# ConsenSys/gnark-crypto

Hardware: AMD Instinct MI355X
Metric: G1 MSM/sec (BN254) (higher is better)
Workload: dtype u32; 1 GPU; BN254 G1 MultiExp 2^20 points, bases+scalars resident in HBM; points=1048576, window_bits=16, windows=8, glv_half_scalars=True, resident_bases=False, parallelism=single GPU

## Files before the change

gnark-crypto_amd/csrc/gmsm_context.h:

```cpp
#pragma once
#include <hip/hip_runtime.h>
#include <atomic>

#include <algorithm>
#include <cstdio>
#include <cstdlib>
#include <chrono>
#include <condition_variable>
#include <memory>
#include <mutex>
#include <string>
#include <thread>
#include <vector>

#include "../../include/gmsm.h"

namespace gmsm {

int fail(int code, const std::string &msg);
void clear_last_error();

#define HIP_TRY(expr)                                                                                        \
    do {                                                                                                     \
        hipError_t e_ = (expr);                                                                              \
// ... 96 lines not shown
        for (auto *b : bufs) any = any || b->ptr;
        if (!any) return;
        int prev = 0;
        (void)hipGetDevice(&prev);
        if (device >= 0) (void)hipSetDevice(device);
        (void)hipDeviceSynchronize();
        for (auto *b : bufs)
            if (b->ptr) (void)hipFree(b->ptr);
        (void)hipSetDevice(prev);
    }
};

struct Workspace {
    hipStream_t stream = nullptr;
    DeviceBuffer upoints, skip;
    DeviceBuffer seg_lvl;
    DeviceBuffer seg_partials, seg_flags, seg_bucket;
    DeviceBuffer parted;
    DeviceBuffer heavy;
    DeviceBuffer long_pieces;
    DeviceBuffer small_sums, small_done;
    DeviceBuffer digits, sorted, blockhist, counts, starts, buckets, partials, totals;
    DeviceBuffer red_pre;
    DeviceBuffer carry;
    hipStream_t mstream = nullptr;
    hipEvent_t ev_buckets = nullptr, ev_merged = nullptr;
    hipStream_t cstream = nullptr;
    hipEvent_t ev_fork = nullptr, ev_conv = nullptr;
    bool conv_pending = false;
    hipEvent_t events[12] = {nullptr};
    bool timed = false;
    int timed_level = 0;
    void *pinned = nullptr;
    size_t pinned_cap = 0;
    DeviceBuffer h2d_points, h2d_scalars;
    DeviceBuffer raw_bytes, flagword;
    DeviceBuffer poly;
    DeviceBuffer lagrange;
    bool busy = false;
    bool ticket = false;
    bool pending = false;
    int pending_group = -1;
    unsigned pending_c = 0;
    uint32_t pending_nw = 0;
    uint32_t pending_gen = 0;
    std::shared_ptr<ResidentBases> bases_ref;
    hipEvent_t dep = nullptr;
    bool uncollected = false;
    hipEvent_t last_use = nullptr;
    hipStream_t last_stream = nullptr;
    bool pending_timed = false;
    size_t trim(size_t keep) {
        DeviceBuffer *all[] = {&upoints, &skip, &seg_lvl, &seg_partials, &seg_flags, &seg_bucket, &parted, &heavy, &long_pieces, &small_sums, &small_done, &digits, &sorted,
                               &blockhist, &counts, &starts, &buckets, &partials, &totals, &red_pre, &carry, &h2d_points,
                               &h2d_scalars, &raw_bytes, &flagword, &poly, &lagrange};
        size_t freed = 0;
        for (DeviceBuffer *b : all)
            if (b->cap > keep) freed += b->release();
        if (pinned && pinned_cap > keep) {
            (void)hipHostFree(pinned);
            pinned = nullptr;
            pinned_cap = 0;
        }
        return freed;
    }
    void destroy() {
        (void)trim(0);
        hipEvent_t *evs[] = {&ev_buckets, &ev_merged, &dep, &last_use, &ev_fork, &ev_conv};
        for (hipEvent_t *e : evs) {
            if (*e) (void)hipEventDestroy(*e);
            *e = nullptr;
        }
        for (auto &e : events) {
            if (e) (void)hipEventDestroy(e);
            e = nullptr;
        }
        if (stream) (void)hipStreamDestroy(stream);
// ... 440 lines not shown
```

gnark-crypto_amd/csrc/gmsm_group.h:

```cpp
#pragma once
#include <algorithm>
#include <cstdlib>
#include <cstring>
#include <thread>
#include <type_traits>
#include <vector>

#include "gmsm_context.h"
#include "gmsm_group_host.h"
#include "gmsm_kernels.h"
#include "gmsm_fixup_q.h"
#include "gmsm_small.h"
#include "gmsm_fixedbase.h"
#include "gmsm_ingest.h"
#include "gmsm_decompress.h"
#include "gmsm_fft.h"
#include "gmsm_poly.h"
#include "gmsm_shplonk.h"
#include "gmsm_fflonk.h"
#include "gmsm_group_fft.h"
#include "gmsm_scale.h"
#include "gmsm_ratio.h"

namespace gmsm {
// ... 332 lines not shown
                                                    "2^(44-c) points for c > 17): use a smaller c or split by point range"
                                                  : "more than 2^27 points in one pipeline run: split the window sums by point range "
                                                    "and add the sets (gmsm_fold_window_sets); the MultiExp entries do this themselves");
        const size_t fine_cnt_bytes = (size_t)4 << fbits;
        const uint32_t stage_cap = fine_cnt_bytes >= 156 * 1024 ? 0u
                                   : (uint32_t)std::min<size_t>(GMSM_TUNE(STAGE_CAP, part_log2 >= 15 ? 39000 : 24576),
                                                              (156 * 1024 - fine_cnt_bytes) / 4);
        if (stage_cap > 40u * 1024u) return fail(GMSM_ERR_ARG, "window geometry: staging slots beyond the fine sort's registers");
        if (fine_cnt_bytes + (size_t)stage_cap * 4 > 160 * 1024)
            return fail(GMSM_ERR_ARG, "window geometry: fine-sort counters exceed the LDS");
        const bool d16 = max_digit_code(plan) < 65536;
        const size_t dsz = d16 ? 2 : 4;

        if ((rc = ws.digits.ensure((size_t)nw * n * dsz))) return rc;
        if ((rc = ws.sorted.ensure((size_t)nw * n * 4))) return rc;
        if ((rc = ws.parted.ensure((size_t)nw * n * 4))) return rc;
        if ((rc = ws.starts.ensure((size_t)nw * (NB + 1) * 4))) return rc;
        if ((rc = ws.buckets.ensure((size_t)nw * NB * REC))) return rc;
        if ((rc = ws.partials.ensure((tot_blk + (size_t)nw * q.nblocks2) * 2 * REC))) return rc;
        const uint32_t T = (uint32_t)(((size_t)NB + ((size_t)1 << q.log2L) - 1) >> q.log2L);
        if ((rc = ws.red_pre.ensure((size_t)nw * T * 2 * REC))) return rc;
        if ((rc = ws.totals.ensure((size_t)nwd * sizeof(Ext)))) return rc;
        if ((rc = ws.ensure_pinned((size_t)nwd * sizeof(Ext)))) return rc;
        if ((rc = ws.blockhist.ensure((size_t)nw * pchunks * nparts * 4))) return rc;
        if ((rc = ws.counts.ensure((size_t)nw * (2 * nparts + 1) * 4))) return rc;
        if ((rc = ws.seg_partials.ensure(tot_thr * 2 * REC))) return rc;
        if ((rc = ws.seg_flags.ensure(tot_thr * 4))) return rc;
        if ((rc = ws.seg_bucket.ensure(tot_thr * 4))) return rc;
        const size_t list_cap = 2 * (tot_thr / FIX_MAXWALK + tot_thr / LONG_PIECE + nw + 16);
        if ((rc = ws.seg_lvl.ensure((size_t)nw * 4 + 16 + list_cap * sizeof(LongChain)))) return rc;
        uint32_t *long_flag = (uint32_t *)ws.seg_lvl.ptr;
        LongChain *long_list = (LongChain *)((char *)ws.seg_lvl.ptr + (((size_t)nw * 4 + 15) / 16) * 16);
        const size_t piece_sums_off = ((list_cap * 4 + 15) / 16) * 16;
        if ((rc = ws.long_pieces.ensure(piece_sums_off + list_cap * REC))) return rc;
        uint32_t *piece_done = (uint32_t *)ws.long_pieces.ptr;
        void *piece_sums = (char *)ws.long_pieces.ptr + piece_sums_off;
        const uint32_t hcap = (uint32_t)std::min<size_t>(nparts, n / ((size_t)stage_cap + 1) + 1);
        const uint32_t scap = (uint32_t)(n / HEAVY_SUB) + hcap;
        const size_t hparts_bytes = (((size_t)nw * hcap * sizeof(HeavyPart) + 15) / 16) * 16, hcount_bytes = (((size_t)nw * 8 + 4 + 15) / 16) * 16;
        if ((rc = ws.heavy.ensure(hparts_bytes + hcount_bytes + ((size_t)nw * scap << fbits) * 4))) return rc;
        HeavyPart *hparts = (HeavyPart *)ws.heavy.ptr;
        uint32_t *hcount = (uint32_t *)((char *)ws.heavy.ptr + hparts_bytes);
        uint32_t *subhist = (uint32_t *)((char *)ws.heavy.ptr + hparts_bytes + hcount_bytes);
        if (nw > HEAVY_MAX_WINDOWS) return fail(GMSM_ERR_ARG, "more than 256 windows in one pipeline run");
        const uint32_t heavy_wg = (uint32_t)std::min<size_t>((size_t)2 * ctx.num_cus, std::max<size_t>((size_t)nw * scap, 1));
        uint32_t *bh = (uint32_t *)ws.blockhist.ptr, *part_base = (uint32_t *)ws.counts.ptr;
// ... 6 lines not shown
        if ((rc = ctx.allow_lds((const void *)k_part_scatter<uint16_t, PART_CHUNK_BIG>, 152 * 1024))) return rc;
        if ((rc = ctx.allow_lds((const void *)k_part_scatter<uint32_t, PART_CHUNK_BIG>, 152 * 1024))) return rc;
        if ((rc = ctx.allow_lds((const void *)k_fine_sort<24>, 160 * 1024))) return rc;
        if ((rc = ctx.allow_lds((const void *)k_fine_sort<40>, 160 * 1024))) return rc;
        if ((rc = ctx.allow_lds((const void *)k_heavy_hist, 128 * 1024))) return rc;
        if ((rc = ctx.allow_lds((const void *)k_heavy_scan, 128 * 1024))) return rc;
        if ((rc = ctx.allow_lds((const void *)k_heavy_place, 128 * 1024))) return rc;
        if ((rc = ctx.allow_lds((const void *)k_fixup_long<U>, (int)(128 * sizeof(QRec<U>))))) return rc;
        if constexpr (FIXUP_QUAD)
            if ((rc = ctx.allow_lds((const void *)k_fixup_seg_q<U>, (int)(128 * sizeof(QRec<U>))))) return rc;
        if ((rc = ctx.allow_lds((const void *)k_combine_q<U, true, COMBINE_N>, (int)((2 * COMBINE_N + 1) * sizeof(QRec<U>))))) return rc;
        if constexpr (COMBINE_WE)
            if ((rc = ctx.allow_lds((const void *)k_combine_we<U, true>, (int)((2 * COMBINE_N + 1) * sizeof(QRec<U>))))) return rc;
        if constexpr (SERIAL_QUAD)
            if ((rc = ctx.allow_lds((const void *)k_reduce_serial_q<U, SERIAL_Q_QUADS>, (int)(3 * SERIAL_Q_QUADS * sizeof(QRec<U>))))) return rc;
        if ((rc = ctx.allow_lds((const void *)k_reduce2_q<U, true>, (int)(2 * RED2_TPB * sizeof(QRec<U>))))) return rc;

        StageTimer timer(ws, !buckets_only || time_range);
        ws.timed = timer.on;
        timer.mark(T_DECOMPOSE, stream);
        const uint8_t *skip = nullptr;
        const void *upoints = nullptr;
        bool forked = false;
        if (resident) {
            upoints = (const char *)(shared ? resident->tables.ptr : resident->upoints.ptr) + resident_offset * AFF_BYTES;
            skip = (const uint8_t *)resident->skip.ptr + resident_offset;
        } else {
            if ((rc = ws.upoints.ensure((glv ? 2 : 1) * n_points * AFF_BYTES))) return rc;
            forked = n_points >= FORK_CONVERT_MIN;
            if (forked && (rc = ws.side_stream(ws.cstream))) return rc;
            hipStream_t cs = forked ? ws.cstream : stream;
            if (forked) {
                HIP_TRY(hipEventRecord(ws.ev_fork, stream));
                HIP_TRY(hipStreamWaitEvent(cs, ws.ev_fork, 0));
            }
            if (glv)
                hipLaunchKernelGGL((k_convert_points_glv<U, Consts>), dim3((unsigned)((n_points + 255) / 256)), dim3(256), 0,
                                   cs, d_points, n_points, ws.upoints.ptr);
            else
                hipLaunchKernelGGL((k_convert_points<U>), dim3((unsigned)((n_points + 255) / 256)), dim3(256), 0,
                                   cs, d_points, n_points, ws.upoints.ptr, (uint8_t *)nullptr);
            if (forked) {
                ws.conv_pending = true;
                HIP_TRY(hipEventRecord(ws.ev_conv, cs));
            }
            upoints = ws.upoints.ptr;
// ... 12 lines not shown
                               (const uint16_t *)digits, n, nparts, fbits, pchunk_len, bh);
        else
            hipLaunchKernelGGL(k_part_hist<uint32_t>, dim3(pchunks, nw), dim3(1024), (size_t)nparts * 4, stream,
                               (const uint32_t *)digits, n, nparts, fbits, pchunk_len, bh);
        timer.mark(T_SCAN, stream);
        if ((size_t)((nparts + 31) / 32) * nw < (size_t)ctx.num_cus && pchunks >= 256)
            hipLaunchKernelGGL(k_part_colscan<32>, dim3((nparts + 31) / 32, nw), dim3(1024), 0, stream, bh, pchunks, nparts, part_pop, hcount + 2 * nw);
        else
            hipLaunchKernelGGL(k_part_colscan<8>, dim3((nparts + 31) / 32, nw), dim3(256), 0, stream, bh, pchunks, nparts, part_pop, hcount + 2 * nw);
        hipLaunchKernelGGL(k_part_rowscan, dim3(nw), dim3(1024), 0, stream, part_pop, nparts, part_base, long_flag, stage_cap, hparts,
                           hcount, hcap);
        timer.mark(T_SCATTER, stream);
        {
            const dim3 grid(pchunks, nw), block(1024);
#define GMSM_SCATTER(D, CH)                                                                                              \
    hipLaunchKernelGGL((k_part_scatter<D, CH>), grid, block, scatter_lds, stream, (const D *)digits, n, nparts, fbits, lidx, \
                       pchunk_len, bh, part_base, parted)
            if (d16 && !big_chunk) GMSM_SCATTER(uint16_t, PART_CHUNK);
            else if (d16) GMSM_SCATTER(uint16_t, PART_CHUNK_BIG);
            else if (!big_chunk) GMSM_SCATTER(uint32_t, PART_CHUNK);
            else GMSM_SCATTER(uint32_t, PART_CHUNK_BIG);
#undef GMSM_SCATTER
        }
        if (stage_cap <= 24u * 1024u)
            hipLaunchKernelGGL(k_fine_sort<24>, dim3(nparts, nw), dim3(1024), ((size_t)4 << fbits) + (size_t)stage_cap * 4, stream,
                               parted, n, NB, fbits, lidx, part_base, sorted, starts, stage_cap);
        else
            hipLaunchKernelGGL(k_fine_sort<40>, dim3(nparts, nw), dim3(1024), ((size_t)4 << fbits) + (size_t)stage_cap * 4, stream,
                               parted, n, NB, fbits, lidx, part_base, sorted, starts, stage_cap);
        if (n > stage_cap) {
            hipLaunchKernelGGL(k_heavy_hist, dim3(heavy_wg), dim3(1024), (size_t)4 << fbits, stream, parted, n, nw, nparts, fbits, lidx,
                               part_base, (const HeavyPart *)hparts, (const uint32_t *)hcount, hcap, scap, subhist);
            hipLaunchKernelGGL(k_heavy_scan, dim3(std::min<uint32_t>(hcap, 64u), nw), dim3(1024), (size_t)4 << fbits, stream, nparts, NB, fbits,
                               part_base, (const HeavyPart *)hparts, (const uint32_t *)hcount, hcap, scap, subhist, starts);
            hipLaunchKernelGGL(k_heavy_place, dim3(heavy_wg), dim3(1024), (size_t)4 << fbits, stream, parted, n, nw, nparts, fbits, lidx,
                               part_base, (const HeavyPart *)hparts, (const uint32_t *)hcount, hcap, scap, (const uint32_t *)subhist, sorted);
        }
        if (forked) {
            HIP_TRY(hipStreamWaitEvent(stream, ws.ev_conv, 0));
            ws.conv_pending = false;
        }
        const auto accumulate = [&](uint32_t k0, uint32_t nk, hipStream_t st) {
            const uint32_t *st_g = starts + (size_t)k0 * (NB + 1);
            const uint32_t *sorted_g = sorted + (size_t)k0 * n;
            char *buckets_g = buckets + (size_t)k0 * NB * REC, *part_g = seg_partials + (size_t)k0 * qa.tpw * 2 * REC;
            if (shared)
                hipLaunchKernelGGL((k_accumulate_seg<U, true>), dim3((qa.tpw + 255) / 256, nk), dim3(256), 0, st, upoints, n, NB,
                                   qa.seg, st_g, sorted_g, buckets_g, part_g, seg_flags + (size_t)k0 * qa.tpw, seg_bucket + (size_t)k0 * qa.tpw,
                                   qa.tpw, (uint32_t)n_points, (uint32_t)resident->n);
            else
                hipLaunchKernelGGL((k_accumulate_seg<U, false>), dim3((qa.tpw + 255) / 256, nk), dim3(256), 0, st, upoints, n, NB,
                                   qa.seg, st_g, sorted_g, buckets_g, part_g, seg_flags + (size_t)k0 * qa.tpw, seg_bucket + (size_t)k0 * qa.tpw,
                                   qa.tpw, 0u, 0u);
        };
        const auto fixup_and_reduce = [&](uint32_t k0, uint32_t nk, size_t list_off, hipStream_t st, bool mark) {
            const uint32_t *st_g = starts + (size_t)k0 * (NB + 1);
            char *buckets_g = buckets + (size_t)k0 * NB * REC, *part_g = seg_partials + (size_t)k0 * qa.tpw * 2 * REC;
            const uint32_t *flags_g = seg_flags + (size_t)k0 * qa.tpw, *pb_g = seg_bucket + (size_t)k0 * qa.tpw;
            uint32_t *cnt_g = long_flag + k0;
            LongChain *list_g = long_list + list_off;
            uint32_t *done_g = piece_done + list_off;
            void *sums_g = (char *)piece_sums + list_off * REC;
            if (shared && n / NB >= 2 * (size_t)qa.seg)
                hipLaunchKernelGGL((k_fixup_bucket<OpsSerial>), dim3((NB + 255) / 256, nk), dim3(256), 0, st, NB, st_g, qa.seg,
                                   (const void *)part_g, qa.tpw, (void *)buckets_g, cnt_g, list_g, done_g, FIX_MAXWALK);
            else if constexpr (FIXUP_QUAD)
                hipLaunchKernelGGL((k_fixup_seg_q<U>), dim3((qa.tpw + 63) / 64, nk), dim3(256), 128 * sizeof(QRec<U>), st, NB,
                                   (const void *)part_g, flags_g, pb_g, qa.tpw, (void *)buckets_g, cnt_g, list_g, done_g, FIX_MAXWALK, st_g, qa.seg);
            else
                hipLaunchKernelGGL((k_fixup_seg<OpsSerial>), dim3((qa.tpw + 255) / 256, nk), dim3(256), 0, st, NB, part_g, flags_g, pb_g,
                                   qa.tpw, buckets_g, cnt_g, list_g, done_g, FIX_MAXWALK, st_g, qa.seg);
            hipLaunchKernelGGL((k_fixup_long<U>), dim3(2 * ctx.num_cus), dim3(256), 128 * sizeof(QRec<U>), st, NB, part_g, pb_g, qa.tpw,
                               buckets_g, (const uint32_t *)cnt_g, (const LongChain *)list_g, done_g, sums_g, st_g, qa.seg);
            if (mark) timer.mark(T_REDUCE, st);
            if (!buckets_only) enqueue_reduce_kernels(ctx, ws, q, T, buckets_g, st_g, nk, NB, st, k0);
        };
        timer.mark(T_ACCUMULATE, stream);
        if (!split) {
            accumulate(0, nw, stream);
            timer.mark(T_FIXUP, stream);
            fixup_and_reduce(0, nw, 0, stream, true);
        } else {
            const uint32_t ha = nw / 2;
            if ((rc = ws.side_stream(ws.mstream))) return rc;
            accumulate(0, ha, stream);
            HIP_TRY(hipEventRecord(ws.ev_buckets, stream));
            HIP_TRY(hipStreamWaitEvent(ws.mstream, ws.ev_buckets, 0));
            fixup_and_reduce(0, ha, 0, ws.mstream, false);
            HIP_TRY(hipEventRecord(ws.ev_merged, ws.mstream));
            accumulate(ha, nw - ha, stream);
            timer.mark(T_FIXUP, stream);
            fixup_and_reduce(ha, nw - ha, list_cap / 2, stream, true);
            HIP_TRY(hipStreamWaitEvent(stream, ws.ev_merged, 0));
        }
        if (!buckets_only && nwd > nw)
            hipLaunchKernelGGL((k_fill_infinity<Ext>), dim3((nwd - nw + 63) / 64), dim3(64), 0, stream, ws.totals.ptr, nw, nwd - nw);
        timer.mark(T_END, stream);
        HIP_TRY(hipGetLastError());
        if (!buckets_only) {
            if (d_out)
                HIP_TRY(hipMemcpyAsync(d_out, ws.totals.ptr, (size_t)nwd * sizeof(Ext), hipMemcpyDeviceToDevice, stream));
            else
                HIP_TRY(hipMemcpyAsync(ws.pinned, ws.totals.ptr, (size_t)nwd * sizeof(Ext), hipMemcpyDeviceToHost, stream));
        }
        if ((rc = end_use(ws, stream))) return rc;
        ws.pending_timed = timer.on;
        return GMSM_OK;
    }

    static uint32_t reduce2_active(uint32_t nlast) {
        uint32_t active = 2;
        while (active < nlast) active <<= 1;
        return active;
    }
    static void reduce_shape(const Context &ctx, uint32_t nw, uint32_t NB, uint32_t out[6]) {
        const Geometry q = plan_geometry(ctx, nw, NB, NB);
        out[0] = q.log2L;
        out[1] = q.nblocks1;
        out[2] = q.nblocks2;
        out[3] = use_combine_we(ctx, q.nblocks1 * nw) ? 2u : 1u;
        out[4] = SERIAL_QUAD ? 1u : 0u;
        out[5] = reduce2_active(q.nblocks2 ? q.nblocks2 : q.nblocks1);
    }

    static void enqueue_reduce_kernels(Context &ctx, Workspace &ws, const Geometry &q, uint32_t T, const void *buckets,
                                       const uint32_t *starts, uint32_t nw, uint32_t NB, hipStream_t stream,
                                       uint32_t k0 = 0 ) {
        constexpr size_t RECB = sizeof(typename OpsSerial::Mem);
        void *red_pre = (char *)ws.red_pre.ptr + (size_t)k0 * T * 2 * RECB;
        void *partials = (char *)ws.partials.ptr + (size_t)k0 * q.nblocks1 * 2 * RECB;
        void *totals = (char *)ws.totals.ptr + (size_t)k0 * sizeof(Ext);
        const uint32_t prescale = q.log2span;
        if constexpr (SERIAL_QUAD)
            hipLaunchKernelGGL((k_reduce_serial_q<U, SERIAL_Q_QUADS>), dim3((T + SERIAL_Q_QUADS - 1) / SERIAL_Q_QUADS, nw), dim3(4 * SERIAL_Q_QUADS),
                               3 * SERIAL_Q_QUADS * sizeof(QRec<U>), stream, buckets, NB, q.log2L, T, starts, red_pre);
        else
            hipLaunchKernelGGL((k_reduce_serial<OpsSerial>), dim3((T + 255) / 256, nw), dim3(256), 0, stream, buckets, NB,
                               q.log2L, T, starts, red_pre);
        const auto combine = [&](const void *in, uint32_t pairs, void *out, uint32_t blocks, uint32_t l2, uint32_t pre) {
            if constexpr (COMBINE_WE) {
                if (use_combine_we(ctx, blocks * nw)) {
                    hipLaunchKernelGGL((k_combine_we<U, true>), dim3(blocks, nw), dim3(4 * COMBINE_N),
                                       (2 * COMBINE_N + 1) * sizeof(QRec<U>), stream, l2, out, pre, in, pairs);
                    return;
                }
            }
            hipLaunchKernelGGL((k_combine_q<U, true, COMBINE_N>), dim3(blocks, nw), dim3(4 * COMBINE_N),
                               (2 * COMBINE_N + 1) * sizeof(QRec<U>), stream, l2, out, pre, in, pairs);
        };
        combine(red_pre, T, partials, q.nblocks1, q.log2L, prescale);
        const void *last = partials;
        uint32_t nlast = q.nblocks1, rest = q.log2span - prescale;
        if (q.nblocks2) {
            constexpr size_t REC = sizeof(typename OpsSerial::Mem);
            void *out2 = (char *)partials + (size_t)nw * q.nblocks1 * 2 * REC;
            uint32_t lgN = 0;
            for (size_t t = COMBINE_N; t > 1; t >>= 1) ++lgN;
            combine(partials, q.nblocks1, out2, q.nblocks2, 0, lgN);
            last = out2;
            nlast = q.nblocks2;
            rest = 0;
        }
        const uint32_t active = reduce2_active(nlast);
        hipLaunchKernelGGL((k_reduce2_q<U, true>), dim3(nw), dim3(4 * active), 2 * active * sizeof(QRec<U>), stream, last, nlast,
                           rest, active, totals);
        (void)ctx;
    }

    static int enqueue_reduce(Context &ctx, Workspace &ws, const void *buckets, const WindowPlan &plan, size_t n_for_geometry,
                              hipStream_t stream) {
        const uint32_t nw = bucket_sets(plan), nwd = plan.nwin_local, NB = plan.nbuckets;
        constexpr size_t REC = sizeof(typename OpsSerial::Mem);
        const Geometry q = plan_geometry(ctx, nw, n_for_geometry, NB);
        const uint32_t T = (uint32_t)(((size_t)NB + ((size_t)1 << q.log2L) - 1) >> q.log2L);
        int rc;
        if ((rc = ws.partials.ensure((size_t)nw * (q.nblocks1 + q.nblocks2) * 2 * REC))) return rc;
        if ((rc = ws.red_pre.ensure((size_t)nw * T * 2 * REC))) return rc;
        if ((rc = ws.totals.ensure((size_t)nwd * sizeof(Ext)))) return rc;
        if ((rc = ws.ensure_pinned((size_t)nwd * sizeof(Ext)))) return rc;
        if ((rc = ctx.allow_lds((const void *)k_combine_q<U, true, COMBINE_N>, (int)((2 * COMBINE_N + 1) * sizeof(QRec<U>))))) return rc;
        if constexpr (COMBINE_WE)
            if ((rc = ctx.allow_lds((const void *)k_combine_we<U, true>, (int)((2 * COMBINE_N + 1) * sizeof(QRec<U>))))) return rc;
        if constexpr (SERIAL_QUAD)
            if ((rc = ctx.allow_lds((const void *)k_reduce_serial_q<U, SERIAL_Q_QUADS>, (int)(3 * SERIAL_Q_QUADS * sizeof(QRec<U>))))) return rc;
        if ((rc = ctx.allow_lds((const void *)k_reduce2_q<U, true>, (int)(2 * RED2_TPB * sizeof(QRec<U>))))) return rc;
        enqueue_reduce_kernels(ctx, ws, q, T, buckets, nullptr, nw, NB, stream);
        if (nwd > nw)
            hipLaunchKernelGGL((k_fill_infinity<Ext>), dim3((nwd - nw + 63) / 64), dim3(64), 0, stream, ws.totals.ptr, nw, nwd - nw);
        HIP_TRY(hipGetLastError());
        HIP_TRY(hipMemcpyAsync(ws.pinned, ws.totals.ptr, (size_t)nwd * sizeof(Ext), hipMemcpyDeviceToHost, stream));
        return GMSM_OK;
    }

    static int normalize_records(Workspace &ws, size_t n, void *d_out) {
        int rc;
        if ((rc = ws.partials.ensure(n * sizeof(U)))) return rc;
        constexpr int K = 32;
        const size_t threads = (n + K - 1) / K;
        hipLaunchKernelGGL((k_batch_normalize<U, INLINE_OPS, K>), dim3((unsigned)((threads + 63) / 64)), dim3(64), 0, ws.stream,
                           ws.buckets.ptr, n, (U *)ws.partials.ptr, d_out);
        HIP_TRY(hipGetLastError());
        return GMSM_OK;
    }

    static int batch_scalar_mul(Context &ctx, Workspace &ws, const uint64_t *base_limbs, const void *d_scalars, size_t n,
                                void *d_out) {
        if (n == 0) return GMSM_OK;
        Aff base;
        memcpy(&base, base_limbs, sizeof base);
        if (base.is_infinity()) {
            HIP_TRY(hipMemsetAsync(d_out, 0, n * AFF_BYTES, ws.stream));
            return GMSM_OK;
        }
// ... 723 lines not shown
```

gnark-crypto_amd/csrc/gmsm_kernels.h:

```cpp
#pragma once
#include <hip/hip_runtime.h>
#include "gmsm_curveu.h"
#include "gmsm_quad.h"

namespace gmsm {

struct WindowPlan {
    uint32_t c;
    uint32_t nwin_total;
    uint32_t nbuckets;
    uint32_t win_first;
    uint32_t win_stride;
    uint32_t nwin_local;
    uint32_t shared;
    uint32_t glv;
};

template <class T>
__device__ __forceinline__ T load_struct(const void *base, size_t index) {
    static_assert(sizeof(T) % 16 == 0, "element size");
    T r;
    const uint4 *src = reinterpret_cast<const uint4 *>(reinterpret_cast<const char *>(base) + index * sizeof(T));
    uint4 *dst = reinterpret_cast<uint4 *>(&r);
#pragma unroll
// ... 850 lines not shown
        }
        const uint32_t c0 = c - lc.piece;
        if (j == 0) quad_rec_store<U>(piece_sums, c, &acc[0], lane);
        __syncthreads();
        if (tid == 0) {
            __threadfence();
            const uint32_t done = __hip_atomic_fetch_add(&piece_done[c0], 1u, __ATOMIC_ACQ_REL, __HIP_MEMORY_SCOPE_AGENT);
            s_last = done + 1u == lc.npieces ? 1u : 0u;
        }
        __syncthreads();
        if (s_last) {
            __threadfence();
            quad_sum_links<U>(acc, stage, lc.npieces, tid, piece_sums, (size_t)c0, 1, ~(size_t)0, false);
            if (j == 0) quad_rec_store<U>(buckets, bucket_index, &acc[0], lane);
        }
        __syncthreads();
    }
}


template <class A>
__global__ void __launch_bounds__(256, 1) k_reduce_serial(const void *__restrict__ buckets, uint32_t nbuckets, uint32_t log2L,
                                                          uint32_t T, const uint32_t *__restrict__ starts,
                                                          void *__restrict__ pre) {
    using E = typename A::Elem;
    const uint32_t g = blockIdx.x * blockDim.x + threadIdx.x, k = blockIdx.y;
    if (g >= T) return;
    const uint32_t L = 1u << log2L, lo = g * L;
    const uint32_t *st = starts ? starts + (size_t)k * (nbuckets + 1) : nullptr;
    E run = A::infinity(), tot = A::infinity();
    auto present = [&](uint32_t b) { return b < nbuckets && (st == nullptr || st[b + 1] > st[b]); };
    bool have_next = present(lo + L - 1);
    E next = A::infinity();
    if (have_next) next = A::load(buckets, (size_t)k * nbuckets + lo + L - 1);
#pragma nounroll
    for (uint32_t j = L; j-- > 0;) {
        const bool have = have_next;
        E B = next;
        have_next = j > 0 && present(lo + j - 1);
        if (have_next) next = A::load(buckets, (size_t)k * nbuckets + lo + j - 1);
        if (have) {
            A::fresh(B);
            A::add(run, B);
        }
        A::add(tot, run);
    }
    A::store(pre, ((size_t)k * T + g) * 2 + 0, run);
    A::store(pre, ((size_t)k * T + g) * 2 + 1, tot);
}

#ifndef GMSM_SERIAL_Q_WAVES
#define GMSM_SERIAL_Q_WAVES 1
#endif
template <class U, int QPB >
__global__ void __launch_bounds__(4 * QPB, GMSM_SERIAL_Q_WAVES) k_reduce_serial_q(const void *__restrict__ buckets, uint32_t nbuckets, uint32_t log2L,
                                                             uint32_t T, const uint32_t *__restrict__ starts,
                                                             void *__restrict__ pre) {
    extern __shared__ __align__(16) unsigned char lds_raw[];
    QRec<U> *run = reinterpret_cast<QRec<U> *>(lds_raw), *tot = run + QPB, *stage = run + 2 * QPB;
    const uint32_t tid = threadIdx.x, j = tid >> 2, lane = tid & 63u, k = blockIdx.y;
    const uint32_t g = blockIdx.x * QPB + j;
    const uint32_t L = 1u << log2L, lo = g * L;
    const uint32_t *st = starts ? starts + (size_t)k * (nbuckets + 1) : nullptr;
    if ((tid & 3u) == 0) {
        run[j].inf = 1u;
        tot[j].inf = 1u;
    }
    quad_lds_fence();
#pragma nounroll
    for (uint32_t jj = L; jj-- > 0;) {
        const uint32_t b = lo + jj;
        const bool present = g < T && b < nbuckets && (st == nullptr || st[b + 1] > st[b]);
        quad_rec_load<U, true>(&stage[j], buckets, (size_t)k * nbuckets + (present ? b : 0), present, lane);
        quad_lds_fence();
        {
            const QAddOps<U> o = quad_add_load<U>(&run[j], &stage[j], lane);
            quad_add_store<U, true>(&run[j], o, present, lane);
        }
        quad_lds_fence();
        {
            const QAddOps<U> o = quad_add_load<U>(&tot[j], &run[j], lane);
            quad_add_store<U, true>(&tot[j], o, g < T, lane);
        }
// ... 63 lines not shown
```

gnark-crypto_amd/csrc/gmsm_quad.h:

```cpp
#pragma once
#include "gmsm_curveu.h"

namespace gmsm {

#if defined(__HIPCC__)

__device__ __forceinline__ void quad_lds_fence() { __builtin_amdgcn_fence(__ATOMIC_ACQ_REL, "wavefront"); }

template <class U>
struct QRec {
    U c[4];
    uint32_t inf;
    uint32_t pad[3];
};

template <class U> struct QF;
template <class P>
struct QF<FpU<P>> {
    using F = FpU<P>;
    template <bool INL> __device__ static __forceinline__ F mul(const F &a, const F &b) { return fmul<INL>(a, b); }
    __device__ static __forceinline__ F sub4(const F &a, const F &b) { return fpu_sub<P, 4>(a, b); }
    __device__ static __forceinline__ F sub16(const F &a, const F &b) { return fpu_sub<P, 16>(a, b); }
    __device__ static __forceinline__ F dbl(const F &a) { return fpu_dbl(a); }
    __device__ static __forceinline__ F triple(const F &a) { return fpu_add(fpu_add(a, a), a); }
// ... 133 lines not shown
    const U *src = reinterpret_cast<const U *>(reinterpret_cast<const char *>(base) + index * sizeof(XYZZL<U>));
    bool inf = true;
    if (present) {
        const U zz = src[2];
        inf = lz_limbs_all_zero(zz);
        U c = src[r];
        if constexpr (FRESH) {
            if (!inf) lz_coord_fresh(c, r);
        }
        dst->c[r] = c;
    }
    if (r == 0u) dst->inf = inf ? 1u : 0u;
}
template <class U>
__device__ __forceinline__ void quad_rec_store(void *base, size_t index, const QRec<U> *src, uint32_t lane) {
    const uint32_t r = lane & 3u;
    U *dst = reinterpret_cast<U *>(reinterpret_cast<char *>(base) + index * sizeof(XYZZL<U>));
    U v = src->c[r];
    if (r == 2u && src->inf) v = lz_zero((const U *)nullptr);
    dst[r] = v;
}

template <class U, bool INL>
__global__ void __launch_bounds__(256) k_reduce2_q(const void *__restrict__ in1, uint32_t nblocks1, uint32_t log2span,
                                                   uint32_t active, void *__restrict__ window_totals) {
    extern __shared__ __align__(16) unsigned char lds_raw[];
    QRec<U> *S = reinterpret_cast<QRec<U> *>(lds_raw), *W = S + active;
    const uint32_t k = blockIdx.x, t = threadIdx.x, j = t >> 2, lane = t & 63u;
    quad_rec_load<U>(&S[j], in1, ((size_t)k * nblocks1 + j) * 2 + 0, j < nblocks1, lane);
    quad_rec_load<U>(&W[j], in1, ((size_t)k * nblocks1 + j) * 2 + 1, j < nblocks1, lane);
    __syncthreads();
#pragma nounroll
    for (uint32_t d = 1; d < active; d <<= 1) {
        const bool act = j + d < active;
        const QAddOps<U> o = quad_add_load<U>(&S[j], &S[act ? j + d : j], lane);
        __syncthreads();
        quad_add_store<U, INL>(&S[j], o, act, lane);
        __syncthreads();
    }
    if (j == 0 && (t & 3u) == 0) S[0].inf = 1u;
    __syncthreads();
#pragma nounroll
    for (uint32_t s = 0; s < log2span; ++s) {
        if (!S[j].inf) quad_dbl_inplace<U, INL>(&S[j], lane);
        __syncthreads();
    }
    {
        const QAddOps<U> o = quad_add_load<U>(&W[j], &S[j], lane);
        quad_add_store<U, INL>(&W[j], o, true, lane);
    }
    __syncthreads();
#pragma nounroll
    for (uint32_t d = active >> 1; d >= 1; d >>= 1) {
        const bool act = j < d;
        const QAddOps<U> o = quad_add_load<U>(&W[j], &W[act ? j + d : j], lane);
        __syncthreads();
        quad_add_store<U, INL>(&W[j], o, act, lane);
        __syncthreads();
    }
    if (t < 4) {
        using T = LzTraits<U>;
        using Mem = XYZZ<typename T::Sat>;
        typename T::Sat *dst = reinterpret_cast<typename T::Sat *>(reinterpret_cast<char *>(window_totals) + (size_t)k * sizeof(Mem));
        typename T::Sat v = T::template to_sat<INL>(W[0].c[t]);
        if (W[0].inf) {
            const Mem inf = Mem::infinity();
            v = t == 0 ? inf.x : t == 1 ? inf.y : t == 2 ? inf.zz : inf.zzz;
        }
        dst[t] = v;
    }
}

template <class U, bool INL, int N>
__global__ void __launch_bounds__(4 * N) k_combine_q(uint32_t log2L, void *__restrict__ out1, uint32_t prescale,
                                                     const void *__restrict__ pre, uint32_t T) {
    extern __shared__ __align__(16) unsigned char lds_raw[];
    QRec<U> *S = reinterpret_cast<QRec<U> *>(lds_raw), *W = S + N, *PARK = S + 2 * N;
    const uint32_t k = blockIdx.y, blk = blockIdx.x, t = threadIdx.x, j = t >> 2, lane = t & 63u;
    const uint32_t g = blk * N + j;
    quad_rec_load<U>(&S[j], pre, ((size_t)k * T + g) * 2 + 0, g < T, lane);
    quad_rec_load<U>(&W[j], pre, ((size_t)k * T + g) * 2 + 1, g < T, lane);
    __syncthreads();
    constexpr uint32_t LG = N == 64 ? 6 : N == 32 ? 5 : N == 16 ? 4 : N == 128 ? 7 : 0;
    static_assert(LG != 0, "N must be 16, 32, 64 or 128");
#pragma nounroll
    for (uint32_t s = 0; s < LG; ++s) {
        const uint32_t d = 1u << s;
        const bool act = j + d < (uint32_t)N;
        const QAddOps<U> o = quad_add_load<U>(&S[j], &S[act ? j + d : j], lane);
        __syncthreads();
        quad_add_store<U, INL>(&S[j], o, act, lane);
        __syncthreads();
    }
    if (j == 0) {
        PARK->c[t & 3u] = S[0].c[t & 3u];
        if ((t & 3u) == 0) {
            PARK->inf = S[0].inf;
            S[0].inf = 1u;
// ... 19 lines not shown
            const uint32_t step = s - n_tree;
            if (j == 0) {
                if (step < log2L) fin_dbl = true;
                else {
                    act = true;
                    X = &W[0];
                    Y = &S[0];
                }
            }
        }
        const bool park_dbl = j == (uint32_t)N - 1 && s >= 1 && dbl_left > 0;
        const QAddOps<U> o = quad_add_load<U>(X, Y, lane);
        __syncthreads();
        quad_add_store<U, INL>(X, o, act, lane);
        if (fin_dbl && !S[0].inf) quad_dbl_inplace<U, INL>(&S[0], lane);
        if (park_dbl) {
            if (!PARK->inf) quad_dbl_inplace<U, INL>(PARK, lane);
        }
        if (s >= 1 && dbl_left > 0) --dbl_left;
        __syncthreads();
    }
    if (j == 0) quad_rec_store<U>(out1, ((size_t)k * gridDim.x + blk) * 2 + 1, &W[0], lane);
    if (j == 1) quad_rec_store<U>(out1, ((size_t)k * gridDim.x + blk) * 2 + 0, PARK, lane);
}

template <class U, bool INL>
__global__ void __launch_bounds__(256) k_combine_we(uint32_t log2L, void *__restrict__ out1, uint32_t prescale,
                                                    const void *__restrict__ pre, uint32_t T) {
    constexpr uint32_t N = 64;
    extern __shared__ __align__(16) unsigned char lds_raw[];
    QRec<U> *S = reinterpret_cast<QRec<U> *>(lds_raw), *W = S + N, *PARK = S + 2 * N;
    const uint32_t k = blockIdx.y, blk = blockIdx.x, t = threadIdx.x, j = t >> 2, lane = t & 63u;
    const uint32_t g0 = blk * N + j;
    quad_rec_load<U>(&S[j], pre, ((size_t)k * T + g0) * 2 + 0, g0 < T, lane);
    quad_rec_load<U>(&W[j], pre, ((size_t)k * T + g0) * 2 + 1, g0 < T, lane);
    __syncthreads();
#pragma nounroll
    for (uint32_t s = 1; s <= 6; ++s) {
        const uint32_t g = 32u >> (s - 1), G = j / g, i = j % g;
        const bool act = G <= s;
        QRec<U> *X = &S[0], *Y = &S[0];
        if (G == 0) {
            const uint32_t l = s - 1;
            X = &S[(2 * i) << l];
            Y = &S[(2 * i + 1) << l];
        } else if (G < s) {
            const uint32_t l = G - 1;
            X = &S[(2 * i + 1) << l];
            Y = &S[(2 * (i + g) + 1) << l];
        } else if (G == s) {
            X = &W[i];
// ... 16 lines not shown
        int op = 0;
        QRec<U> *X = &S[0], *Y = &S[0];
        if (j < 3) {
            if (s == 0) { op = 1; X = &S[2u << (2 * j)]; }
            else if (s == 1) { op = 2; X = &S[1u << (2 * j)]; Y = &S[2u << (2 * j)]; }
            else if (s == 2 || s == 3) { if (j >= 1) { op = 1; X = &S[j == 1 ? 4 : 16]; } }
            else if (s == 4) { if (j == 0) { op = 2; X = &S[1]; Y = &S[4]; } else if (j == 2) { op = 1; X = &S[16]; } }
            else if (s == 5) { if (j == 2) { op = 1; X = &S[16]; } }
            else if (s == 6) { if (j == 0) { op = 2; X = &S[1]; Y = &S[16]; } }
            else if (s < 7 + log2L) { if (j == 0) { op = 1; X = &S[1]; } }
            else if (j == 0) { op = 2; X = &W[0]; Y = &S[1]; }
        }
        const bool park_dbl = j == 15 && dbl_left > 0;
        const QAddOps<U> o = quad_add_load<U>(X, Y, lane);
        __syncthreads();
        quad_add_store<U, INL>(X, o, op == 2, lane);
        if (op == 1 && !X->inf) quad_dbl_inplace<U, INL>(X, lane);
        if (park_dbl && !PARK->inf) quad_dbl_inplace<U, INL>(PARK, lane);
        if (dbl_left > 0) --dbl_left;
        __syncthreads();
    }
    if (j == 0) quad_rec_store<U>(out1, ((size_t)k * gridDim.x + blk) * 2 + 1, &W[0], lane);
    if (j == 1) quad_rec_store<U>(out1, ((size_t)k * gridDim.x + blk) * 2 + 0, PARK, lane);
}

#endif

}
```

Before: 560.7 MSM/s.

## Fuse final window reduction into combine kernel via last-block arrival counter

Adds a per-window arrival counter so that the last combine block to finish performs the final reduce2 step and writes window totals directly, removing the separate k_reduce2_q launch when few blocks remain. Totals are written straight into pinned host memory, which drops the device-to-host memcpy. The heavy-partition sort kernels are also moved onto a side stream so they overlap with the fine sort. These changes add atomics, thread fences and a write to pinned memory from the kernel, which trades launch and copy overhead for extra cross-block synchronisation.

```diff
diff --git a/gnark-crypto_amd/csrc/gmsm_context.h b/gnark-crypto_amd/csrc/gmsm_context.h
--- a/gnark-crypto_amd/csrc/gmsm_context.h
+++ b/gnark-crypto_amd/csrc/gmsm_context.h
@@ -142,6 +142,7 @@
     DeviceBuffer small_sums, small_done;
     DeviceBuffer digits, sorted, blockhist, counts, starts, buckets, partials, totals;
     DeviceBuffer red_pre;
+    DeviceBuffer arrive;
     DeviceBuffer carry;
     hipStream_t mstream = nullptr;
     hipEvent_t ev_buckets = nullptr, ev_merged = nullptr;
@@ -172,7 +173,7 @@
     bool pending_timed = false;
     size_t trim(size_t keep) {
         DeviceBuffer *all[] = {&upoints, &skip, &seg_lvl, &seg_partials, &seg_flags, &seg_bucket, &parted, &heavy, &long_pieces, &small_sums, &small_done, &digits, &sorted,
-                               &blockhist, &counts, &starts, &buckets, &partials, &totals, &red_pre, &carry, &h2d_points,
+                               &blockhist, &counts, &starts, &buckets, &partials, &totals, &red_pre, &arrive, &carry, &h2d_points,
                                &h2d_scalars, &raw_bytes, &flagword, &poly, &lagrange};
         size_t freed = 0;
         for (DeviceBuffer *b : all)
diff --git a/gnark-crypto_amd/csrc/gmsm_group.h b/gnark-crypto_amd/csrc/gmsm_group.h
--- a/gnark-crypto_amd/csrc/gmsm_group.h
+++ b/gnark-crypto_amd/csrc/gmsm_group.h
@@ -378,6 +378,8 @@
         if ((rc = ws.red_pre.ensure((size_t)nw * T * 2 * REC))) return rc;
         if ((rc = ws.totals.ensure((size_t)nwd * sizeof(Ext)))) return rc;
         if ((rc = ws.ensure_pinned((size_t)nwd * sizeof(Ext)))) return rc;
+        if ((rc = ensure_arrive(ws, nw))) return rc;
+        void *const totals_dst = d_out ? ws.totals.ptr : ws.pinned;
         if ((rc = ws.blockhist.ensure((size_t)nw * pchunks * nparts * 4))) return rc;
         if ((rc = ws.counts.ensure((size_t)nw * (2 * nparts + 1) * 4))) return rc;
         if ((rc = ws.seg_partials.ensure(tot_thr * 2 * REC))) return rc;
@@ -430,6 +432,9 @@
         const uint8_t *skip = nullptr;
         const void *upoints = nullptr;
         bool forked = false;
+        const bool heavy = n > stage_cap;
+        const bool fork_heavy = heavy && n_points >= FORK_CONVERT_MIN;
+        if (fork_heavy && (rc = ws.side_stream(ws.cstream))) return rc;
         if (resident) {
             upoints = (const char *)(shared ? resident->tables.ptr : resident->upoints.ptr) + resident_offset * AFF_BYTES;
             skip = (const uint8_t *)resident->skip.ptr + resident_offset;
@@ -488,21 +493,29 @@
             else GMSM_SCATTER(uint32_t, PART_CHUNK_BIG);
 #undef GMSM_SCATTER
         }
+        const auto heavy_sort = [&](hipStream_t st) {
+            hipLaunchKernelGGL(k_heavy_hist, dim3(heavy_wg), dim3(1024), (size_t)4 << fbits, st, parted, n, nw, nparts, fbits, lidx,
+                               part_base, (const HeavyPart *)hparts, (const uint32_t *)hcount, hcap, scap, subhist);
+            hipLaunchKernelGGL(k_heavy_scan, dim3(std::min<uint32_t>(hcap, 64u), nw), dim3(1024), (size_t)4 << fbits, st, nparts, NB, fbits,
+                               part_base, (const HeavyPart *)hparts, (const uint32_t *)hcount, hcap, scap, subhist, starts);
+            hipLaunchKernelGGL(k_heavy_place, dim3(heavy_wg), dim3(1024), (size_t)4 << fbits, st, parted, n, nw, nparts, fbits, lidx,
+                               part_base, (const HeavyPart *)hparts, (const uint32_t *)hcount, hcap, scap, (const uint32_t *)subhist, sorted);
+        };
+        if (fork_heavy) {
+            HIP_TRY(hipEventRecord(ws.ev_fork, stream));
+            HIP_TRY(hipStreamWaitEvent(ws.cstream, ws.ev_fork, 0));
+            heavy_sort(ws.cstream);
+            ws.conv_pending = true;
+            HIP_TRY(hipEventRecord(ws.ev_conv, ws.cstream));
+        }
         if (stage_cap <= 24u * 1024u)
             hipLaunchKernelGGL(k_fine_sort<24>, dim3(nparts, nw), dim3(1024), ((size_t)4 << fbits) + (size_t)stage_cap * 4, stream,
                                parted, n, NB, fbits, lidx, part_base, sorted, starts, stage_cap);
         else
             hipLaunchKernelGGL(k_fine_sort<40>, dim3(nparts, nw), dim3(1024), ((size_t)4 << fbits) + (size_t)stage_cap * 4, stream,
                                parted, n, NB, fbits, lidx, part_base, sorted, starts, stage_cap);
-        if (n > stage_cap) {
-            hipLaunchKernelGGL(k_heavy_hist, dim3(heavy_wg), dim3(1024), (size_t)4 << fbits, stream, parted, n, nw, nparts, fbits, lidx,
-                               part_base, (const HeavyPart *)hparts, (const uint32_t *)hcount, hcap, scap, subhist);
-            hipLaunchKernelGGL(k_heavy_scan, dim3(std::min<uint32_t>(hcap, 64u), nw), dim3(1024), (size_t)4 << fbits, stream, nparts, NB, fbits,
-                               part_base, (const HeavyPart *)hparts, (const uint32_t *)hcount, hcap, scap, subhist, starts);
-            hipLaunchKernelGGL(k_heavy_place, dim3(heavy_wg), dim3(1024), (size_t)4 << fbits, stream, parted, n, nw, nparts, fbits, lidx,
-                               part_base, (const HeavyPart *)hparts, (const uint32_t *)hcount, hcap, scap, (const uint32_t *)subhist, sorted);
-        }
-        if (forked) {
+        if (heavy && !fork_heavy) heavy_sort(stream);
+        if (forked || fork_heavy) {
             HIP_TRY(hipStreamWaitEvent(stream, ws.ev_conv, 0));
             ws.conv_pending = false;
         }
@@ -539,7 +552,7 @@
             hipLaunchKernelGGL((k_fixup_long<U>), dim3(2 * ctx.num_cus), dim3(256), 128 * sizeof(QRec<U>), st, NB, part_g, pb_g, qa.tpw,
                                buckets_g, (const uint32_t *)cnt_g, (const LongChain *)list_g, done_g, sums_g, st_g, qa.seg);
             if (mark) timer.mark(T_REDUCE, st);
-            if (!buckets_only) enqueue_reduce_kernels(ctx, ws, q, T, buckets_g, st_g, nk, NB, st, k0);
+            if (!buckets_only) enqueue_reduce_kernels(ctx, ws, q, T, buckets_g, st_g, nk, NB, st, totals_dst, k0);
         };
         timer.mark(T_ACCUMULATE, stream);
         if (!split) {
@@ -560,15 +573,11 @@
             HIP_TRY(hipStreamWaitEvent(stream, ws.ev_merged, 0));
         }
         if (!buckets_only && nwd > nw)
-            hipLaunchKernelGGL((k_fill_infinity<Ext>), dim3((nwd - nw + 63) / 64), dim3(64), 0, stream, ws.totals.ptr, nw, nwd - nw);
+            hipLaunchKernelGGL((k_fill_infinity<Ext>), dim3((nwd - nw + 63) / 64), dim3(64), 0, stream, totals_dst, nw, nwd - nw);
         timer.mark(T_END, stream);
         HIP_TRY(hipGetLastError());
-        if (!buckets_only) {
-            if (d_out)
-                HIP_TRY(hipMemcpyAsync(d_out, ws.totals.ptr, (size_t)nwd * sizeof(Ext), hipMemcpyDeviceToDevice, stream));
-            else
-                HIP_TRY(hipMemcpyAsync(ws.pinned, ws.totals.ptr, (size_t)nwd * sizeof(Ext), hipMemcpyDeviceToHost, stream));
-        }
+        if (!buckets_only && d_out)
+            HIP_TRY(hipMemcpyAsync(d_out, ws.totals.ptr, (size_t)nwd * sizeof(Ext), hipMemcpyDeviceToDevice, stream));
         if ((rc = end_use(ws, stream))) return rc;
         ws.pending_timed = timer.on;
         return GMSM_OK;
@@ -589,40 +598,53 @@
         out[5] = reduce2_active(q.nblocks2 ? q.nblocks2 : q.nblocks1);
     }
 
+#ifndef GMSM_FUSE_LAST_MAX
+#define GMSM_FUSE_LAST_MAX 4
+#endif
+    static constexpr uint32_t FUSE_LAST_MAX = GMSM_FUSE_LAST_MAX;
+    static int ensure_arrive(Workspace &ws, uint32_t nw) { return ws.arrive.ensure((((size_t)nw * 4 + 15) / 16) * 16); }
+
     static void enqueue_reduce_kernels(Context &ctx, Workspace &ws, const Geometry &q, uint32_t T, const void *buckets,
-                                       const uint32_t *starts, uint32_t nw, uint32_t NB, hipStream_t stream,
+                                       const uint32_t *starts, uint32_t nw, uint32_t NB, hipStream_t stream, void *totals_dst,
                                        uint32_t k0 = 0 ) {
         constexpr size_t RECB = sizeof(typename OpsSerial::Mem);
         void *red_pre = (char *)ws.red_pre.ptr + (size_t)k0 * T * 2 * RECB;
         void *partials = (char *)ws.partials.ptr + (size_t)k0 * q.nblocks1 * 2 * RECB;
-        void *totals = (char *)ws.totals.ptr + (size_t)k0 * sizeof(Ext);
+        void *totals = (char *)totals_dst + (size_t)k0 * sizeof(Ext);
+        uint32_t *arrive = (uint32_t *)ws.arrive.ptr + k0;
         const uint32_t prescale = q.log2span;
         if constexpr (SERIAL_QUAD)
             hipLaunchKernelGGL((k_reduce_serial_q<U, SERIAL_Q_QUADS>), dim3((T + SERIAL_Q_QUADS - 1) / SERIAL_Q_QUADS, nw), dim3(4 * SERIAL_Q_QUADS),
-                               3 * SERIAL_Q_QUADS * sizeof(QRec<U>), stream, buckets, NB, q.log2L, T, starts, red_pre);
+                               3 * SERIAL_Q_QUADS * sizeof(QRec<U>), stream, buckets, NB, q.log2L, T, starts, red_pre, arrive);
         else
             hipLaunchKernelGGL((k_reduce_serial<OpsSerial>), dim3((T + 255) / 256, nw), dim3(256), 0, stream, buckets, NB,
-                               q.log2L, T, starts, red_pre);
-        const auto combine = [&](const void *in, uint32_t pairs, void *out, uint32_t blocks, uint32_t l2, uint32_t pre) {
+                               q.log2L, T, starts, red_pre, arrive);
+        const auto combine = [&](const void *in, uint32_t pairs, void *out, uint32_t blocks, uint32_t l2, uint32_t pre,
+                                 uint32_t rest_dbl, void *fin) {
             if constexpr (COMBINE_WE) {
                 if (use_combine_we(ctx, blocks * nw)) {
                     hipLaunchKernelGGL((k_combine_we<U, true>), dim3(blocks, nw), dim3(4 * COMBINE_N),
-                                       (2 * COMBINE_N + 1) * sizeof(QRec<U>), stream, l2, out, pre, in, pairs);
+                                       (2 * COMBINE_N + 1) * sizeof(QRec<U>), stream, l2, out, pre, in, pairs, rest_dbl, fin, arrive);
                     return;
                 }
             }
             hipLaunchKernelGGL((k_combine_q<U, true, COMBINE_N>), dim3(blocks, nw), dim3(4 * COMBINE_N),
-                               (2 * COMBINE_N + 1) * sizeof(QRec<U>), stream, l2, out, pre, in, pairs);
+                               (2 * COMBINE_N + 1) * sizeof(QRec<U>), stream, l2, out, pre, in, pairs, rest_dbl, fin, arrive);
         };
-        combine(red_pre, T, partials, q.nblocks1, q.log2L, prescale);
+        const auto fused = [&](uint32_t blocks) { return blocks <= FUSE_LAST_MAX; };
         const void *last = partials;
         uint32_t nlast = q.nblocks1, rest = q.log2span - prescale;
+        const bool fin1 = !q.nblocks2 && fused(q.nblocks1);
+        combine(red_pre, T, partials, q.nblocks1, q.log2L, prescale, rest, fin1 ? totals : nullptr);
+        if (fin1) return;
         if (q.nblocks2) {
             constexpr size_t REC = sizeof(typename OpsSerial::Mem);
             void *out2 = (char *)partials + (size_t)nw * q.nblocks1 * 2 * REC;
             uint32_t lgN = 0;
             for (size_t t = COMBINE_N; t > 1; t >>= 1) ++lgN;
-            combine(partials, q.nblocks1, out2, q.nblocks2, 0, lgN);
+            const bool fin2 = fused(q.nblocks2);
+            combine(partials, q.nblocks1, out2, q.nblocks2, 0, lgN, 0, fin2 ? totals : nullptr);
+            if (fin2) return;
             last = out2;
             nlast = q.nblocks2;
             rest = 0;
@@ -630,7 +652,6 @@
         const uint32_t active = reduce2_active(nlast);
         hipLaunchKernelGGL((k_reduce2_q<U, true>), dim3(nw), dim3(4 * active), 2 * active * sizeof(QRec<U>), stream, last, nlast,
                            rest, active, totals);
-        (void)ctx;
     }
 
     static int enqueue_reduce(Context &ctx, Workspace &ws, const void *buckets, const WindowPlan &plan, size_t n_for_geometry,
@@ -644,17 +665,17 @@
         if ((rc = ws.red_pre.ensure((size_t)nw * T * 2 * REC))) return rc;
         if ((rc = ws.totals.ensure((size_t)nwd * sizeof(Ext)))) return rc;
         if ((rc = ws.ensure_pinned((size_t)nwd * sizeof(Ext)))) return rc;
+        if ((rc = ensure_arrive(ws, nw))) return rc;
         if ((rc = ctx.allow_lds((const void *)k_combine_q<U, true, COMBINE_N>, (int)((2 * COMBINE_N + 1) * sizeof(QRec<U>))))) return rc;
         if constexpr (COMBINE_WE)
             if ((rc = ctx.allow_lds((const void *)k_combine_we<U, true>, (int)((2 * COMBINE_N + 1) * sizeof(QRec<U>))))) return rc;
         if constexpr (SERIAL_QUAD)
             if ((rc = ctx.allow_lds((const void *)k_reduce_serial_q<U, SERIAL_Q_QUADS>, (int)(3 * SERIAL_Q_QUADS * sizeof(QRec<U>))))) return rc;
         if ((rc = ctx.allow_lds((const void *)k_reduce2_q<U, true>, (int)(2 * RED2_TPB * sizeof(QRec<U>))))) return rc;
-        enqueue_reduce_kernels(ctx, ws, q, T, buckets, nullptr, nw, NB, stream);
+        enqueue_reduce_kernels(ctx, ws, q, T, buckets, nullptr, nw, NB, stream, ws.pinned);
         if (nwd > nw)
-            hipLaunchKernelGGL((k_fill_infinity<Ext>), dim3((nwd - nw + 63) / 64), dim3(64), 0, stream, ws.totals.ptr, nw, nwd - nw);
+            hipLaunchKernelGGL((k_fill_infinity<Ext>), dim3((nwd - nw + 63) / 64), dim3(64), 0, stream, ws.pinned, nw, nwd - nw);
         HIP_TRY(hipGetLastError());
-        HIP_TRY(hipMemcpyAsync(ws.pinned, ws.totals.ptr, (size_t)nwd * sizeof(Ext), hipMemcpyDeviceToHost, stream));
         return GMSM_OK;
     }
 
diff --git a/gnark-crypto_amd/csrc/gmsm_kernels.h b/gnark-crypto_amd/csrc/gmsm_kernels.h
--- a/gnark-crypto_amd/csrc/gmsm_kernels.h
+++ b/gnark-crypto_amd/csrc/gmsm_kernels.h
@@ -896,9 +896,11 @@
 template <class A>
 __global__ void __launch_bounds__(256, 1) k_reduce_serial(const void *__restrict__ buckets, uint32_t nbuckets, uint32_t log2L,
                                                           uint32_t T, const uint32_t *__restrict__ starts,
-                                                          void *__restrict__ pre) {
+                                                          void *__restrict__ pre,
+                                                          uint32_t *__restrict__ arrive ) {
     using E = typename A::Elem;
     const uint32_t g = blockIdx.x * blockDim.x + threadIdx.x, k = blockIdx.y;
+    if (arrive != nullptr && g == 0) arrive[k] = 0;
     if (g >= T) return;
     const uint32_t L = 1u << log2L, lo = g * L;
     const uint32_t *st = starts ? starts + (size_t)k * (nbuckets + 1) : nullptr;
@@ -929,10 +931,12 @@
 template <class U, int QPB >
 __global__ void __launch_bounds__(4 * QPB, GMSM_SERIAL_Q_WAVES) k_reduce_serial_q(const void *__restrict__ buckets, uint32_t nbuckets, uint32_t log2L,
                                                              uint32_t T, const uint32_t *__restrict__ starts,
-                                                             void *__restrict__ pre) {
+                                                             void *__restrict__ pre,
+                                                             uint32_t *__restrict__ arrive ) {
     extern __shared__ __align__(16) unsigned char lds_raw[];
     QRec<U> *run = reinterpret_cast<QRec<U> *>(lds_raw), *tot = run + QPB, *stage = run + 2 * QPB;
     const uint32_t tid = threadIdx.x, j = tid >> 2, lane = tid & 63u, k = blockIdx.y;
+    if (arrive != nullptr && blockIdx.x == 0 && tid == 0) arrive[k] = 0;
     const uint32_t g = blockIdx.x * QPB + j;
     const uint32_t L = 1u << log2L, lo = g * L;
     const uint32_t *st = starts ? starts + (size_t)k * (nbuckets + 1) : nullptr;
diff --git a/gnark-crypto_amd/csrc/gmsm_quad.h b/gnark-crypto_amd/csrc/gmsm_quad.h
--- a/gnark-crypto_amd/csrc/gmsm_quad.h
+++ b/gnark-crypto_amd/csrc/gmsm_quad.h
@@ -179,6 +179,52 @@
 }
 
 template <class U, bool INL>
+__device__ __forceinline__ void reduce2_steps(QRec<U> *S, QRec<U> *W, uint32_t active, uint32_t log2span, uint32_t t) {
+    const uint32_t j = t >> 2, lane = t & 63u;
+    const bool live = j < active;
+    const uint32_t jl = live ? j : 0u;
+#pragma nounroll
+    for (uint32_t d = 1; d < active; d <<= 1) {
+        const bool act = live && j + d < active;
+        const QAddOps<U> o = quad_add_load<U>(&S[jl], &S[act ? j + d : jl], lane);
+        __syncthreads();
+        quad_add_store<U, INL>(&S[jl], o, act, lane);
+        __syncthreads();
+    }
+    if (j == 0 && (t & 3u) == 0) S[0].inf = 1u;
+    __syncthreads();
+#pragma nounroll
+    for (uint32_t s = 0; s < log2span; ++s) {
+        if (live && !S[jl].inf) quad_dbl_inplace<U, INL>(&S[jl], lane);
+        __syncthreads();
+    }
+    {
+        const QAddOps<U> o = quad_add_load<U>(&W[jl], &S[jl], lane);
+        quad_add_store<U, INL>(&W[jl], o, live, lane);
+    }
+    __syncthreads();
+#pragma nounroll
+    for (uint32_t d = active >> 1; d >= 1; d >>= 1) {
+        const bool act = live && j < d;
+        const QAddOps<U> o = quad_add_load<U>(&W[jl], &W[act ? j + d : jl], lane);
+        __syncthreads();
+        quad_add_store<U, INL>(&W[jl], o, act, lane);
+        __syncthreads();
+    }
+}
+template <class U, bool INL>
+__device__ __forceinline__ void reduce2_store_total(const QRec<U> *R, void *window_totals, uint32_t k, uint32_t t) {
+    if (t < 4) {
+        using T = LzTraits<U>;
+        using Mem = XYZZ<typename T::Sat>;
+        typename T::Sat *dst = reinterpret_cast<typename T::Sat *>(reinterpret_cast<char *>(window_totals) + (size_t)k * sizeof(Mem));
+        typename T::Sat v = T::template to_sat<INL>(R->c[t]);
+        if (R->inf) v = t < 2 ? T::Sat::one() : T::Sat::zero();
+        dst[t] = v;
+    }
+}
+
+template <class U, bool INL>
 __global__ void __launch_bounds__(256) k_reduce2_q(const void *__restrict__ in1, uint32_t nblocks1, uint32_t log2span,
                                                    uint32_t active, void *__restrict__ window_totals) {
     extern __shared__ __align__(16) unsigned char lds_raw[];
@@ -187,50 +233,46 @@
     quad_rec_load<U>(&S[j], in1, ((size_t)k * nblocks1 + j) * 2 + 0, j < nblocks1, lane);
     quad_rec_load<U>(&W[j], in1, ((size_t)k * nblocks1 + j) * 2 + 1, j < nblocks1, lane);
     __syncthreads();
-#pragma nounroll
-    for (uint32_t d = 1; d < active; d <<= 1) {
-        const bool act = j + d < active;
-        const QAddOps<U> o = quad_add_load<U>(&S[j], &S[act ? j + d : j], lane);
-        __syncthreads();
-        quad_add_store<U, INL>(&S[j], o, act, lane);
-        __syncthreads();
-    }
-    if (j == 0 && (t & 3u) == 0) S[0].inf = 1u;
-    __syncthreads();
-#pragma nounroll
-    for (uint32_t s = 0; s < log2span; ++s) {
-        if (!S[j].inf) quad_dbl_inplace<U, INL>(&S[j], lane);
-        __syncthreads();
-    }
-    {
-        const QAddOps<U> o = quad_add_load<U>(&W[j], &S[j], lane);
-        quad_add_store<U, INL>(&W[j], o, true, lane);
-    }
-    __syncthreads();
-#pragma nounroll
-    for (uint32_t d = active >> 1; d >= 1; d >>= 1) {
-        const bool act = j < d;
-        const QAddOps<U> o = quad_add_load<U>(&W[j], &W[act ? j + d : j], lane);
-        __syncthreads();
-        quad_add_store<U, INL>(&W[j], o, act, lane);
-        __syncthreads();
-    }
-    if (t < 4) {
-        using T = LzTraits<U>;
-        using Mem = XYZZ<typename T::Sat>;
-        typename T::Sat *dst = reinterpret_cast<typename T::Sat *>(reinterpret_cast<char *>(window_totals) + (size_t)k * sizeof(Mem));
-        typename T::Sat v = T::template to_sat<INL>(W[0].c[t]);
-        if (W[0].inf) {
-            const Mem inf = Mem::infinity();
-            v = t == 0 ? inf.x : t == 1 ? inf.y : t == 2 ? inf.zz : inf.zzz;
-        }
-        dst[t] = v;
-    }
+    reduce2_steps<U, INL>(S, W, active, log2span, t);
+    reduce2_store_total<U, INL>(&W[0], window_totals, k, t);
+}
+
+template <class U, bool INL>
+__device__ __forceinline__ void combine_finish(QRec<U> *lds, uint32_t n_rec, const QRec<U> *Wblk, void *out1, uint32_t log2span,
+                                               void *window_totals, uint32_t *arrive, uint32_t k, uint32_t t) {
+    const uint32_t nlast = gridDim.x;
+    if (nlast == 1) {
+        reduce2_store_total<U, INL>(Wblk, window_totals, k, t);
+        return;
+    }
+    QRec<U> *FLAG = lds + n_rec - 1;
+    __threadfence();
+    __syncthreads();
+    if (t == 0) {
+        __threadfence();
+        const uint32_t before = __hip_atomic_fetch_add(&arrive[k], 1u, __ATOMIC_RELAXED, __HIP_MEMORY_SCOPE_AGENT);
+        FLAG->pad[0] = before + 1u == nlast ? 1u : 0u;
+    }
+    __syncthreads();
+    if (FLAG->pad[0] == 0u) return;
+    __threadfence();
+    uint32_t active = 2;
+    while (active < nlast) active <<= 1;
+    QRec<U> *S = lds, *W = lds + active;
+    const uint32_t j = t >> 2, lane = t & 63u;
+    if (j < active) {
+        quad_rec_load<U>(&S[j], out1, ((size_t)k * nlast + j) * 2 + 0, j < nlast, lane);
+        quad_rec_load<U>(&W[j], out1, ((size_t)k * nlast + j) * 2 + 1, j < nlast, lane);
+    }
+    __syncthreads();
+    reduce2_steps<U, INL>(S, W, active, log2span, t);
+    reduce2_store_total<U, INL>(&W[0], window_totals, k, t);
 }
 
 template <class U, bool INL, int N>
 __global__ void __launch_bounds__(4 * N) k_combine_q(uint32_t log2L, void *__restrict__ out1, uint32_t prescale,
-                                                     const void *__restrict__ pre, uint32_t T) {
+                                                     const void *__restrict__ pre, uint32_t T, uint32_t rest,
+                                                     void *window_totals, uint32_t *arrive) {
     extern __shared__ __align__(16) unsigned char lds_raw[];
     QRec<U> *S = reinterpret_cast<QRec<U> *>(lds_raw), *W = S + N, *PARK = S + 2 * N;
     const uint32_t k = blockIdx.y, blk = blockIdx.x, t = threadIdx.x, j = t >> 2, lane = t & 63u;
@@ -296,11 +338,13 @@
     }
     if (j == 0) quad_rec_store<U>(out1, ((size_t)k * gridDim.x + blk) * 2 + 1, &W[0], lane);
     if (j == 1) quad_rec_store<U>(out1, ((size_t)k * gridDim.x + blk) * 2 + 0, PARK, lane);
+    if (window_totals != nullptr) combine_finish<U, INL>(S, 2 * N + 1, &W[0], out1, rest, window_totals, arrive, k, t);
 }
 
 template <class U, bool INL>
 __global__ void __launch_bounds__(256) k_combine_we(uint32_t log2L, void *__restrict__ out1, uint32_t prescale,
-                                                    const void *__restrict__ pre, uint32_t T) {
+                                                    const void *__restrict__ pre, uint32_t T, uint32_t rest,
+                                                    void *window_totals, uint32_t *arrive) {
     constexpr uint32_t N = 64;
     extern __shared__ __align__(16) unsigned char lds_raw[];
     QRec<U> *S = reinterpret_cast<QRec<U> *>(lds_raw), *W = S + N, *PARK = S + 2 * N;
@@ -363,6 +407,7 @@
     }
     if (j == 0) quad_rec_store<U>(out1, ((size_t)k * gridDim.x + blk) * 2 + 1, &W[0], lane);
     if (j == 1) quad_rec_store<U>(out1, ((size_t)k * gridDim.x + blk) * 2 + 0, PARK, lane);
+    if (window_totals != nullptr) combine_finish<U, INL>(S, 2 * N + 1, &W[0], out1, rest, window_totals, arrive, k, t);
 }
 
 #endif
```

After: 547.0 MSM/s. -2.4%, worse.
